# wamuumu/query-recommendation-system

Measured on AMD Instinct MI355X. Metric: MinHash signatures/sec through the whole hot path (signatures -> LSH candidates -> pair scoring -> top-K), higher is better.
Workload: dtype u16/int32 MinHash values, uint64 keys and pairs (integer); float64 cosine

## Files before the change

### include/qrlsh.h

```cpp
#ifndef QRLSH_H
#define QRLSH_H

#include <stddef.h>
#include <stdint.h>

#ifdef __cplusplus
extern "C" {
#endif

#define QRLSH_OK 0
#define QRLSH_EINVAL (-1)
#define QRLSH_EHIP (-2)
#define QRLSH_EUNSUPPORTED (-3)
#define QRLSH_EWORKSPACE (-4)

#define QRLSH_PERM_U16 0
#define QRLSH_PERM_I32 1

#define QRLSH_SIG_I32 0
#define QRLSH_SIG_U16 1

#define QRLSH_SORT_MIX 1u
#define QRLSH_SORT_IOTA 2u
#define QRLSH_SORT_FOLD 4u
// ... 63 lines not shown
int qrlsh_region_unique_count(const uint64_t *grouped, int64_t n, int32_t group_bits, int32_t id_bits, int64_t nids,
                              uint64_t *tmp, void *workspace, size_t workspace_bytes, uint64_t *total_overflow_out,
                              void *stream);
int qrlsh_region_unique_fill(const uint64_t *tmp, int64_t n, int32_t group_bits, int64_t nids, const void *workspace,
                             uint64_t *out, void *stream);

size_t qrlsh_pair_regions_words(int64_t n, int64_t nids, int32_t group_bits, double words_per_query);
size_t qrlsh_pair_regions_tmp_words(int64_t n, int64_t nids, int32_t group_bits, double words_per_query);
int64_t qrlsh_pair_regions_cap(int64_t n, int64_t nids, int32_t group_bits, double words_per_query);
int64_t qrlsh_pair_regions_count(int64_t n, int64_t nids, int32_t group_bits, double words_per_query);
int qrlsh_pair_regions_scatter(const uint64_t *words, int64_t n, int32_t group_bits, int64_t nids, double words_per_query,
                               uint64_t *tmp_regions, uint64_t *regions, uint32_t *counts, uint32_t *overflow_out,
                               void *stream);
int qrlsh_region_unique_count_regions(const uint64_t *regions, const uint32_t *counts, int64_t cap, int64_t n,
                                      int32_t group_bits, int32_t id_bits, int64_t nids, uint64_t *tmp, void *workspace,
                                      size_t workspace_bytes, uint64_t *total_overflow_out, void *stream);
int qrlsh_region_unique_count_regions3(const uint64_t *regions, const uint32_t *counts, int64_t cap, int64_t n,
                                       int32_t group_bits, int32_t id_bits, int64_t nids, uint64_t *tmp, void *workspace,
                                       size_t workspace_bytes, const uint32_t *scatter_overflow, uint64_t *out3,
                                       void *stream);
int qrlsh_pair_regions_scatter32(const uint64_t *words, int64_t n, int32_t group_bits, int32_t id_bits, int64_t nids,
                                 double words_per_query, uint64_t *tmp_regions, uint32_t *regions, uint32_t *counts,
                                 uint32_t *overflow_out, void *stream);
int qrlsh_region_unique_count_regions32(const uint32_t *regions, const uint32_t *counts, int64_t cap, int64_t n,
                                        int32_t group_bits, int32_t id_bits, int64_t nids, uint64_t *tmp, void *workspace,
                                        size_t workspace_bytes, const uint32_t *scatter_overflow, uint64_t *out3,
                                        void *stream);

int qrlsh_row_norms(const int32_t *sig, int64_t nq, int32_t P, int64_t *norm2_out, void *stream);
int qrlsh_verify_pairs(const void *sig, int32_t sig_dtype, int32_t P, int32_t b, const uint64_t *pairs,
                       int64_t n, uint8_t *flags_out, void *stream);
int qrlsh_score_pairs(const void *sig, int32_t sig_dtype, const int64_t *norm2, int32_t P,
                      const uint64_t *pairs, int64_t n, int32_t *milli_out, double *cos_out,
                      uint64_t *edge_out, int32_t id_bits, uint32_t *edge_dst_out, void *stream);

int qrlsh_topk_count(const uint64_t *sorted_edges, int64_t n_edges, int32_t K, int32_t id_bits,
                     void *workspace, size_t workspace_bytes, uint64_t *total_out, void *stream);
int qrlsh_topk_fill(const uint64_t *sorted_edges, const uint32_t *sorted_dst, int64_t n_edges, int32_t K,
                    int32_t id_bits, const void *workspace, int32_t *src_out, int32_t *dst_out,
                    int32_t *milli_out, void *stream);
int qrlsh_topk_fill_based(const uint64_t *sorted_edges, const uint32_t *sorted_dst, int64_t n_edges, int32_t K,
                          int32_t id_bits, int64_t src_base, const void *workspace, int32_t *src_out,
                          int32_t *dst_out, int32_t *milli_out, void *stream);

int qrlsh_score_pairs_rev(const void *sig, int32_t sig_dtype, const int64_t *norm2, int32_t P,
                          const uint64_t *pairs, int64_t n, int32_t *milli_out, uint64_t *rev_out, int32_t id_bits,
// ... 113 lines not shown
```

### query-recommendation-system_amd/csrc/sort.hip

```cpp
#include "common.h"

constexpr int SORT_THREADS = 256;
constexpr int SORT_IPT = 16;
constexpr int SORT_TILE = SORT_THREADS * SORT_IPT;
constexpr int RADIX = 256;

__device__ static inline int xcd_tile(int bid, int ntiles) {
  const int q = ntiles >> 3, r = ntiles & 7, x = bid & 7, y = bid >> 3;
  return (x < r ? x * (q + 1) : r * (q + 1) + (x - r) * q) + y;
}

enum { SM_PLAIN = 0, SM_MIX = 1, SM_FOLD = 2, SM_OWNER = 3, SM_HOST = 4 };
template <int MODE> __device__ static inline uint32_t digit_of(uint64_t key, int shift, uint32_t fold = 0) {
  if (MODE == SM_OWNER || MODE == SM_HOST) {
    const uint64_t o = MODE == SM_HOST ? qr_pair_host(key, fold) : (key >> shift) / fold;
    return o < RADIX ? (uint32_t)o : RADIX - 1;
  }
  uint64_t x = key;
  if (MODE == SM_MIX) x = qr_mix64(key);
  if (MODE == SM_FOLD) x = ((key >> 32) << fold) | (key & ((1ull << fold) - 1ull));
  return (uint32_t)(x >> shift) & (RADIX - 1);
}

template <int MIX>
// ... 304 lines not shown
  const int ntile = (int)min((int64_t)SORT_TILE, n - tbase);
#pragma unroll
  for (int k = 0; k < SORT_IPT; ++k) {
    const int p = k * SORT_THREADS + threadIdx.x;
    if (p < ntile) {
      const uint64_t kk = skey[p];
      keys_out[boff + gdelta[digit_of<MODE>(kk, shift, fold)] + (uint32_t)p] = kk;
    }
  }
}

struct PartPool {
  uint64_t *keys;
  uint32_t *vals;
  unsigned long long *cursor;
  uint32_t cap;
  uint4 *runs;
  unsigned long long *nruns;
  uint32_t runs_max;
  uint32_t *fill;
  uint32_t slot_base;
};

#ifndef QR_PS_IPT
#define QR_PS_IPT 16
#endif
constexpr int PS_IPT = QR_PS_IPT;
constexpr int PS_TILE = SORT_THREADS * PS_IPT;
constexpr int PS_WGS = PS_IPT <= 16 ? 3 : 2;
template <bool LEVEL2>
__global__ __launch_bounds__(SORT_THREADS, PS_WGS) void part_scatter_atomic_kernel(
    const uint64_t *__restrict__ keys_in, const uint32_t *__restrict__ vals_in, uint64_t *__restrict__ keys_out,
    uint32_t *__restrict__ vals_out, int64_t n_in, int ntiles, int shift, uint32_t dmask,
    uint32_t *__restrict__ cursors, uint32_t cap, uint32_t *__restrict__ overflow, uint64_t ek,
    const uint32_t *__restrict__ in_counts, uint32_t in_cap, int64_t chunk_len, int64_t chunk_stride,
    int64_t band_stride, PartPool pool) {
  __shared__ uint32_t cnt[RADIX];
  __shared__ uint32_t lsum[SORT_THREADS / WAVE];
  __shared__ uint32_t gdelta[RADIX];
  __shared__ uint8_t gok[RADIX];
  __shared__ uint64_t skey[PS_TILE];
  __shared__ uint32_t sval[PS_TILE];
  const int tile = LEVEL2 ? (int)blockIdx.x : xcd_tile(blockIdx.x, ntiles), batch = blockIdx.y;
  const int lane = threadIdx.x & (WAVE - 1), w = threadIdx.x >> 6;
  const int64_t n = LEVEL2 ? (int64_t)min(in_counts[batch], in_cap) : n_in;
  const int64_t tbase = (int64_t)tile * PS_TILE;
  if (tbase >= n) return;
  cnt[threadIdx.x] = 0;
  __syncthreads();
  const size_t boff = LEVEL2 ? (size_t)batch * in_cap : (size_t)batch * (size_t)(band_stride ? band_stride : n);
  const bool chunked = !LEVEL2 && chunk_len > 0 && chunk_len < n;
  const int64_t wbase = tbase + (int64_t)w * (WAVE * PS_IPT);
  const uint32_t nd = dmask + 1u;
  uint64_t key[PS_IPT];
  uint32_t val[PS_IPT];
  uint32_t dr[PS_IPT];
#pragma unroll
  for (int k = 0; k < PS_IPT; ++k) {
    const int64_t idx = wbase + (int64_t)k * WAVE + lane;
    const size_t at = chunked ? boff + (size_t)(idx / chunk_len) * chunk_stride + (size_t)(idx % chunk_len) : boff + idx;
    key[k] = idx < n ? keys_in[at] : ek;
    val[k] = LEVEL2 ? (idx < n ? vals_in[boff + idx] : 0u) : (uint32_t)idx;
  }
#pragma unroll
  for (int k = 0; k < PS_IPT; ++k) {
    const int64_t idx = wbase + (int64_t)k * WAVE + lane;
    const bool valid = idx < n && (LEVEL2 || key[k] != ek);
    if (!LEVEL2) key[k] = qr_mix64(key[k]);
    const uint32_t d = (uint32_t)(key[k] >> shift) & dmask;
    dr[k] = valid ? (d << 16) | atomicAdd(&cnt[d], 1u) : 0xFFFFFFFFu;
  }
  __syncthreads();
  const uint32_t tc = cnt[threadIdx.x];
  const uint32_t gb = tc ? atomicAdd(&cursors[(size_t)batch * nd + threadIdx.x], tc) : 0u;
  uint32_t lstart;
  {
    uint32_t linc = tc;
#pragma unroll
    for (int k = 1; k < WAVE; k <<= 1) {
      const uint32_t lo = __shfl_up(linc, k, WAVE);
      if (lane >= k) linc += lo;
    }
    if (lane == WAVE - 1) lsum[w] = linc;
    __syncthreads();
    lstart = linc - tc;
#pragma unroll
    for (int k = 0; k < SORT_THREADS / WAVE; ++k)
      if (k < w) lstart += lsum[k];
    cnt[threadIdx.x] = lstart;
  }
  __syncthreads();
#pragma unroll
  for (int k = 0; k < PS_IPT; ++k) {
    if (dr[k] != 0xFFFFFFFFu) {
      const uint32_t lp = cnt[dr[k] >> 16] + (dr[k] & 0xFFFFu);
      skey[lp] = key[k];
      sval[lp] = val[k];
    }
  }
  {
    const int d = threadIdx.x;
    uint32_t where = gb + tc <= cap ? 1u : 0u;
    uint32_t delta = (uint32_t)d * cap + gb - lstart;
    if (!where) {
      if (pool.keys) {
        const unsigned long long pb =
            __hip_atomic_fetch_add(pool.cursor, (unsigned long long)tc, __ATOMIC_RELAXED, __HIP_MEMORY_SCOPE_AGENT);
        if (pb + tc <= (unsigned long long)pool.cap) {
          const unsigned long long ri = __hip_atomic_fetch_add(pool.nruns, 1ull, __ATOMIC_RELAXED, __HIP_MEMORY_SCOPE_AGENT);
          if (ri < (unsigned long long)pool.runs_max) {
            const uint32_t slot = pool.slot_base + (uint32_t)batch * nd + (uint32_t)d;
            pool.runs[ri] = make_uint4(slot, tc, (uint32_t)pb, 0u);
            atomicMin(&pool.fill[slot], gb);
            where = 2u;
            delta = (uint32_t)pb - lstart;
          }
        }
      }
      if (!where) atomicOr(overflow, 1u);
    }
    gok[d] = (uint8_t)where;
    gdelta[d] = delta;
  }
  __syncthreads();
  uint32_t nstaged = 0;
#pragma unroll
  for (int k = 0; k < SORT_THREADS / WAVE; ++k) nstaged += lsum[k];
  const size_t obase = (size_t)batch * nd * cap;
#pragma unroll
  for (int k = 0; k < PS_IPT; ++k) {
    const uint32_t p = k * SORT_THREADS + threadIdx.x;
    if (p < nstaged) {
      const uint64_t x = skey[p];
      const uint32_t d = (uint32_t)(x >> shift) & dmask;
      const uint32_t where = gok[d];
      if (where == 1u) {
        const size_t dst = obase + (uint32_t)(gdelta[d] + p);
        keys_out[dst] = x;
        vals_out[dst] = sval[p];
      } else if (where == 2u) {
        const uint32_t dst = gdelta[d] + p;
        pool.keys[dst] = x;
        pool.vals[dst] = sval[p];
      }
    }
  }
}

#ifndef QR_PG_IPT
#define QR_PG_IPT 32
#endif
constexpr int PG_IPT = QR_PG_IPT;
constexpr int PG_TILE = SORT_THREADS * PG_IPT;
constexpr int PG_WGS = PG_IPT <= 16 ? 4 : PG_IPT <= 40 ? 2 : 1;
template <bool LEVEL2, typename W>
__global__ __launch_bounds__(SORT_THREADS, PG_WGS) void pair_group_scatter_kernel(
    const uint64_t *__restrict__ in, W *__restrict__ out, int64_t n_in, int ntiles, int shift, uint32_t dmask,
    uint32_t *__restrict__ cursors, uint32_t cap, uint32_t *__restrict__ overflow, const uint32_t *__restrict__ in_counts,
    uint32_t in_cap, int gbits, int jbits) {
  __shared__ uint32_t cnt[RADIX];
  __shared__ uint32_t lsum[SORT_THREADS / WAVE];
  __shared__ uint32_t gdelta[RADIX];
  __shared__ uint8_t gok[RADIX];
  __shared__ uint64_t skey[PG_TILE];
  const int tile = LEVEL2 ? (int)blockIdx.x : xcd_tile(blockIdx.x, ntiles), batch = blockIdx.y;
  const int lane = threadIdx.x & (WAVE - 1), w = threadIdx.x >> 6;
  const int64_t n = LEVEL2 ? (int64_t)min(in_counts[batch], in_cap) : n_in;
  const int64_t tbase = (int64_t)tile * PG_TILE;
  if (tbase >= n) return;
  cnt[threadIdx.x] = 0;
  __syncthreads();
  const size_t boff = LEVEL2 ? (size_t)batch * in_cap : 0;
  const int64_t wbase = tbase + (int64_t)w * (WAVE * PG_IPT);
  const uint32_t nd = dmask + 1u;
  uint64_t key[PG_IPT];
  uint32_t dr[PG_IPT];
#pragma unroll
  for (int k = 0; k < PG_IPT; ++k) {
    const int64_t idx = wbase + (int64_t)k * WAVE + lane;
    key[k] = idx < n ? in[boff + idx] : 0ull;
  }
#pragma unroll
  for (int k = 0; k < PG_IPT; ++k) {
    const int64_t idx = wbase + (int64_t)k * WAVE + lane;
    const uint32_t d = (uint32_t)(key[k] >> shift) & dmask;
    dr[k] = idx < n ? (d << 16) | atomicAdd(&cnt[d], 1u) : 0xFFFFFFFFu;
  }
  __syncthreads();
  const uint32_t tc = cnt[threadIdx.x];
  const uint32_t gb = tc ? atomicAdd(&cursors[(size_t)batch * nd + threadIdx.x], tc) : 0u;
  uint32_t lstart;
  {
    uint32_t linc = tc;
#pragma unroll
    for (int k = 1; k < WAVE; k <<= 1) {
      const uint32_t lo = __shfl_up(linc, k, WAVE);
      if (lane >= k) linc += lo;
    }
    if (lane == WAVE - 1) lsum[w] = linc;
    __syncthreads();
    lstart = linc - tc;
#pragma unroll
    for (int k = 0; k < SORT_THREADS / WAVE; ++k)
      if (k < w) lstart += lsum[k];
    cnt[threadIdx.x] = lstart;
  }
  __syncthreads();
#pragma unroll
  for (int k = 0; k < PG_IPT; ++k)
    if (dr[k] != 0xFFFFFFFFu) skey[cnt[dr[k] >> 16] + (dr[k] & 0xFFFFu)] = key[k];
  {
    const int d = threadIdx.x;
    const bool ok = (uint64_t)gb + tc <= cap;
    if (!ok) atomicOr(overflow, 1u);
    gok[d] = ok;
    gdelta[d] = (uint32_t)d * cap + gb - lstart;
  }
  __syncthreads();
  uint32_t nstaged = 0;
#pragma unroll
  for (int k = 0; k < SORT_THREADS / WAVE; ++k) nstaged += lsum[k];
  const size_t obase = (size_t)batch * nd * cap;
#pragma unroll
  for (int k = 0; k < PG_IPT; ++k) {
    const uint32_t p = k * SORT_THREADS + threadIdx.x;
    if (p < nstaged) {
      const uint64_t x = skey[p];
      const uint32_t d = (uint32_t)(x >> shift) & dmask;
      if (gok[d]) {
        if constexpr (sizeof(W) == 4)
          out[obase + (uint32_t)(gdelta[d] + p)] =
              (((uint32_t)(x >> 32) & ((1u << gbits) - 1u)) << jbits) | ((uint32_t)x & ((1u << jbits) - 1u));
        else
          out[obase + (uint32_t)(gdelta[d] + p)] = x;
      }
    }
  }
}

struct PairRegions {
  int rbits, ra, rb;
  int64_t nregions;
  int64_t na;
  uint32_t cap_a, cap_b;
};
static PairRegions pair_regions(int64_t n, int64_t nids, int group_bits, double words_per_query) {
  PairRegions r;
  const int64_t nr = (nids + (1ll << group_bits) - 1) >> group_bits;
  r.rbits = 1;
  while ((1ll << r.rbits) < nr) ++r.rbits;
  r.rb = r.rbits <= 8 ? r.rbits : (r.rbits + 1) / 2;
  r.ra = r.rbits - r.rb;
  r.na = (nr + (1ll << r.rb) - 1) >> r.rb;
  r.nregions = r.na << r.rb;
  double per = (double)n / (double)(nr > 0 ? nr : 1);
  const double hint = words_per_query * (double)(1ll << group_bits);
  if (hint > per) per = hint;
  const double cb = 3.0 * per + 4096.0;
  const double ca = r.ra ? 2.5 * per * (double)(1ll << r.rb) + 65536.0 : 0.0;
  r.cap_b = (uint32_t)(cb > 4.0e9 ? 4.0e9 : cb);
// ... 30 lines not shown

template <typename W>
static int pair_regions_scatter_impl(const uint64_t *words, int64_t n, int32_t group_bits, int32_t id_bits, int64_t nids,
                                     double words_per_query, uint64_t *tmp_regions, W *regions, uint32_t *counts,
                                     uint32_t *overflow_out, void *stream) {
  QR_CHECK_ARG(n >= 0 && n < (1ll << 32) && nids > 0 && group_bits >= 0 && group_bits <= 8 && counts && overflow_out,
               "qrlsh_pair_regions_scatter: bad arguments");
  hipStream_t st = static_cast<hipStream_t>(stream);
  const PairRegions r = pair_regions(n > 0 ? n : 1, nids, group_bits, words_per_query);
  QR_CHECK_ARG(r.rbits <= 16 && r.na <= RADIX, "qrlsh_pair_regions_scatter: %d region bits", r.rbits);
  QR_CHECK_ARG(pair_regions_fit_u32(r),
               "qrlsh_pair_regions_scatter: regions reach 2^32 words (na * cap_a = %llu, 2^rb * cap_b = %llu; need both < 2^32)",
               (unsigned long long)r.na * r.cap_a, (unsigned long long)r.cap_b << r.rb);
  if (hipMemsetAsync(counts, 0, ((size_t)r.nregions + RADIX) * sizeof(uint32_t), st) != hipSuccess ||
      hipMemsetAsync(overflow_out, 0, sizeof(uint32_t), st) != hipSuccess) {
    qrlsh_set_error("qrlsh_pair_regions_scatter: hipMemsetAsync failed");
    return QRLSH_EHIP;
  }
  if (n == 0) return QRLSH_OK;
  QR_CHECK_ARG(words && regions && (r.ra == 0 || tmp_regions), "qrlsh_pair_regions_scatter: null pointer");
  const int ntiles = (int)ceil_div64(n, PG_TILE);
  const int sh = 32 + group_bits;
  if (r.ra == 0) {
    QR_LAUNCH("pair_group", (pair_group_scatter_kernel<false, W>), dim3(ntiles, 1), dim3(SORT_THREADS), 0, st, words, regions, n,
              ntiles, sh, (1u << r.rb) - 1u, counts, r.cap_b, overflow_out, (const uint32_t *)nullptr, 0u, (int)group_bits,
              (int)id_bits);
  } else {
    uint32_t *cur_a = counts + r.nregions;
    QR_LAUNCH("pair_group", (pair_group_scatter_kernel<false, uint64_t>), dim3(ntiles, 1), dim3(SORT_THREADS), 0, st, words,
              tmp_regions, n, ntiles, sh + r.rb, (1u << r.ra) - 1u, cur_a, r.cap_a, overflow_out, (const uint32_t *)nullptr, 0u,
              0, 0);
    QR_LAUNCH("pair_group", (pair_group_scatter_kernel<true, W>), dim3((unsigned)ceil_div64(r.cap_a, PG_TILE), (unsigned)r.na),
              dim3(SORT_THREADS), 0, st, (const uint64_t *)tmp_regions, regions, (int64_t)0, 0, sh, (1u << r.rb) - 1u, counts,
              r.cap_b, overflow_out, (const uint32_t *)cur_a, r.cap_a, (int)group_bits, (int)id_bits);
  }
  QR_LAUNCH_CHECK("qrlsh_pair_regions_scatter");
  return QRLSH_OK;
}

QRLSH_EXPORT int qrlsh_pair_regions_scatter(const uint64_t *words, int64_t n, int32_t group_bits, int64_t nids,
                                            double words_per_query, uint64_t *tmp_regions, uint64_t *regions,
                                            uint32_t *counts, uint32_t *overflow_out, void *stream) {
  return pair_regions_scatter_impl<uint64_t>(words, n, group_bits, 0, nids, words_per_query, tmp_regions, regions, counts,
                                             overflow_out, stream);
}

QRLSH_EXPORT int qrlsh_pair_regions_scatter32(const uint64_t *words, int64_t n, int32_t group_bits, int32_t id_bits,
                                              int64_t nids, double words_per_query, uint64_t *tmp_regions, uint32_t *regions,
                                              uint32_t *counts, uint32_t *overflow_out, void *stream) {
  QR_CHECK_ARG(group_bits >= 0 && group_bits <= 8 && id_bits >= 1 && id_bits <= 31 && nids > 0 && nids <= (1ll << id_bits) &&
                   (group_bits + id_bits < 32 || (group_bits + id_bits == 32 && nids < (1ll << id_bits))),
               "qrlsh_pair_regions_scatter32: group_bits=%d / id_bits=%d / nids=%lld do not fit a 32-bit value", group_bits,
               id_bits, (long long)nids);
  return pair_regions_scatter_impl<uint32_t>(words, n, group_bits, id_bits, nids, words_per_query, tmp_regions, regions,
                                             counts, overflow_out, stream);
}
// ... 902 lines not shown
  pool.cap = (uint32_t)pool_records(nq, b);
  pool.runs = w.runs;
  pool.runs_max = POOL_RUNS;
  pool.fill = w.fill;
  pool.slot_base = 0;
  PartPool no_pool = pool;
  no_pool.keys = nullptr;
  no_pool.vals = nullptr;
  if (hipMemsetAsync(w.fill, 0xFF, ((size_t)b << T) * sizeof(uint32_t), st) != hipSuccess ||
      hipMemsetAsync(w.poolctl, 0, 16, st) != hipSuccess) {
    qrlsh_set_error("qrlsh_bucket_pairs_emit: hipMemsetAsync failed");
    return QRLSH_EHIP;
  }
  constexpr int MAX_GROUPS = EMIT_MAX_GROUPS;
  unsigned long long *nbig0 = reinterpret_cast<unsigned long long *>(w.big);
  uint64_t *biglist0 = w.big + MAX_GROUPS;
  const uint64_t slots = (uint64_t)b << T;
  if (hipMemsetAsync(nbig0, 0, MAX_GROUPS * sizeof(unsigned long long), st) != hipSuccess) {
    qrlsh_set_error("qrlsh_bucket_pairs_emit: hipMemsetAsync failed");
    return QRLSH_EHIP;
  }
  const bool small_parts = two && small_form(nq, T);
  const int ntiles = (int)ceil_div64(nq, PS_TILE);
  const int64_t band_words = key_band_stride ? key_band_stride : nq;
  const int GROUPS = (int64_t)b * nq >= (64ll << 20) ? MAX_GROUPS : 1;
  const int per = (b + GROUPS - 1) / GROUPS;
  const int ngroups = (b + per - 1) / per;
  const uint64_t list_room = (slots - MAX_GROUPS) / (uint64_t)ngroups;
  const uint32_t big_max = (uint32_t)(list_room < FIN_BIG_LIST ? list_room : FIN_BIG_LIST);
  if (ngroups > 1 && hipMemsetAsync(w.runs, 0, (size_t)POOL_RUNS * sizeof(uint4), st) != hipSuccess) {
    qrlsh_set_error("qrlsh_bucket_pairs_emit: hipMemsetAsync failed");
    return QRLSH_EHIP;
  }
  hipStream_t aux = nullptr;
  int gi = 0;
  for (int g0 = 0; g0 < b; g0 += per, ++gi) {
    const int nb = (b - g0 < per) ? b - g0 : per;
    hipStream_t s = (aux && (gi & 1)) ? aux : st;
    uint64_t *biglist = biglist0 + (size_t)gi * big_max;
    unsigned long long *nbig = nbig0 + gi;
    uint64_t *k1 = two ? tmp_keys : part_keys;
    uint32_t *v1 = two ? tmp_ids : part_ids;
    pool.slot_base = (uint32_t)((size_t)g0 << T);
    BigDesc *desc = w.desc + (size_t)gi * FIN_BIG_LIST;
    QR_PART_SCATTER(false, dim3(ntiles, nb), dim3(SORT_THREADS), 0, s, keys + (size_t)g0 * band_words,
                    (const uint32_t *)nullptr, k1 + ((size_t)g0 << c1) * cap1, v1 + ((size_t)g0 << c1) * cap1, nq,
                    ntiles, 64 - c1, (1u << c1) - 1u, cur1 + ((size_t)g0 << c1), cap1, ovf, qr_empty_key(r),
                    (const uint32_t *)nullptr, 0u, key_chunk, key_chunk_stride, key_band_stride, two ? no_pool : pool);
    if (two)
      QR_PART_SCATTER(true, dim3((unsigned)ceil_div64(cap1, PS_TILE), nb << c1), dim3(SORT_THREADS), 0, s,
                      (const uint64_t *)tmp_keys + ((size_t)g0 << c1) * cap1,
                      (const uint32_t *)tmp_ids + ((size_t)g0 << c1) * cap1, part_keys + ((size_t)g0 << T) * cap2,
                      part_ids + ((size_t)g0 << T) * cap2, (int64_t)0, 0, 64 - T, lowmask, cur2 + ((size_t)g0 << T),
                      cap2, ovf, qr_empty_key(r), (const uint32_t *)cur1 + ((size_t)g0 << c1), cap1, (int64_t)0,
                      (int64_t)0, (int64_t)0, pool);
    if (gi == 0 && b > per) aux = qr_aux_fork(st);
    if (small_parts && T >= 12)
      QR_LAUNCH("bucket_emit", bucket_finish_packed_kernel, dim3(nparts, nb), dim3(FIN_PK_THREADS), 0, s,
                (const uint64_t *)part_keys + ((size_t)g0 << T) * cap2, (const uint32_t *)part_ids + ((size_t)g0 << T) * cap2,
                nparts, total_overflow_out, ovf, pairs_out, capacity, (const uint32_t *)cur2 + ((size_t)g0 << T), cap2, biglist,
                nbig, big_max, (uint32_t)((size_t)g0 << T));
    else if (small_parts)
      QR_LAUNCH("bucket_emit", (bucket_finish_kernel<FIN_SMALL_THREADS, FIN_SMALL_CAP>), dim3(nparts, nb),
                dim3(FIN_SMALL_THREADS), 0, s, (const uint64_t *)part_keys + ((size_t)g0 << T) * cap2,
                (const uint32_t *)part_ids + ((size_t)g0 << T) * cap2, nparts, ekx,
                total_overflow_out, ovf, pairs_out, capacity, (const uint32_t *)cur2 + ((size_t)g0 << T), cap2, biglist, nbig,
                big_max, (uint32_t)((size_t)g0 << T));
    else
      QR_LAUNCH("bucket_emit", (bucket_finish_kernel<>), dim3(nparts, nb), dim3(FIN_THREADS), 0, s,
                (const uint64_t *)part_keys + ((size_t)g0 << T) * cap2, (const uint32_t *)part_ids + ((size_t)g0 << T) * cap2,
                nparts, ekx, total_overflow_out, ovf, pairs_out, capacity,
                (const uint32_t *)cur2 + ((size_t)g0 << T), cap2, biglist, nbig, big_max, (uint32_t)((size_t)g0 << T));
    QR_LAUNCH("bucket_emit_big", bucket_big_gather_kernel, dim3(64), dim3(256), 0, s, (const uint64_t *)biglist,
              (const unsigned long long *)nbig, big_max, desc, (const uint64_t *)part_keys, (const uint32_t *)part_ids,
              (const uint32_t *)cur2, cap2, pool, g_big_limit, ovf);
    QR_LAUNCH("bucket_emit_big", bucket_finish_big_kernel, dim3(FIN_BIG_GRID), dim3(FIN_THREADS), 0, s,
// ... 10 lines not shown
```

### query-recommendation-system_amd/qrlsh/_lib.py

```python
import ctypes
import os

_HERE = os.path.dirname(os.path.abspath(__file__))
LIB_PATH = os.environ.get("QRLSH_LIB", os.path.join(_HERE, "libqrlsh.so"))

QRLSH_OK = 0
QRLSH_EINVAL = -1
QRLSH_EHIP = -2
QRLSH_EUNSUPPORTED = -3
QRLSH_EWORKSPACE = -4

PERM_U16 = 0
PERM_I32 = 1
SIG_I32 = 0
SIG_U16 = 1
SORT_MIX = 1
SORT_IOTA = 2
SORT_FOLD = 4
SORT_OWNER = 8
SORT_HOST = 16
SUM_PAIRWISE = 0
SUM_SEQUENTIAL = 1
RECOMMEND_MAX_K = 1024
INDEX_MAX_K = 256
# ... 23 lines not shown
    "qrlsh_bucket_part_words": (_sz, [_i64, _i32, _i32]),
    "qrlsh_set_big_part_limit": (_i64, [_i64]),
    "qrlsh_set_score_runs": (_i32, [_i32]),
    "qrlsh_bucket_tmp_words": (_sz, [_i64, _i32, _i32]),
    "qrlsh_bucket_pairs_emit": (ctypes.c_int, [_vp, _vp, _vp, _vp, _vp, _i64, _i32, _i32, _i32, _vp, _sz, _vp, _u64, _vp, _vp]),
    "qrlsh_compact_workspace_bytes": (_sz, [_i64]),
    "qrlsh_row_unique_workspace_bytes": (_sz, [_i64]),
    "qrlsh_row_unique_count": (ctypes.c_int, [_vp, _i64, _i32, _i32, _vp, _vp, _sz, _vp, _vp]),
    "qrlsh_row_unique_fill": (ctypes.c_int, [_vp, _i64, _vp, _vp, _vp]),
    "qrlsh_region_unique_workspace_bytes": (_sz, [_i64, _i32]),
    "qrlsh_region_unique_count": (ctypes.c_int, [_vp, _i64, _i32, _i32, _i64, _vp, _vp, _sz, _vp, _vp]),
    "qrlsh_region_unique_fill": (ctypes.c_int, [_vp, _i64, _i32, _i64, _vp, _vp, _vp]),
    "qrlsh_region_unique_count_regions": (ctypes.c_int, [_vp, _vp, _i64, _i64, _i32, _i32, _i64, _vp, _vp, _sz, _vp, _vp]),
    "qrlsh_region_unique_count_regions3": (ctypes.c_int, [_vp, _vp, _i64, _i64, _i32, _i32, _i64, _vp, _vp, _sz, _vp, _vp,
                                                          _vp]),
    "qrlsh_region_unique_count_regions32": (ctypes.c_int, [_vp, _vp, _i64, _i64, _i32, _i32, _i64, _vp, _vp, _sz, _vp, _vp,
                                                           _vp]),
    "qrlsh_pair_regions_scatter32": (ctypes.c_int, [_vp, _i64, _i32, _i32, _i64, ctypes.c_double, _vp, _vp, _vp, _vp, _vp]),
    "qrlsh_pair_regions_words": (_sz, [_i64, _i64, _i32, ctypes.c_double]),
    "qrlsh_pair_regions_tmp_words": (_sz, [_i64, _i64, _i32, ctypes.c_double]),
    "qrlsh_pair_regions_cap": (_i64, [_i64, _i64, _i32, ctypes.c_double]),
    "qrlsh_pair_regions_count": (_i64, [_i64, _i64, _i32, ctypes.c_double]),
    "qrlsh_pair_regions_scatter": (ctypes.c_int, [_vp, _i64, _i32, _i64, ctypes.c_double, _vp, _vp, _vp, _vp, _vp]),
    "qrlsh_unique_count": (ctypes.c_int, [_vp, _i64, _vp, _sz, _vp, _vp]),
    "qrlsh_unique_fill": (ctypes.c_int, [_vp, _i64, _vp, _vp, _vp]),
    "qrlsh_row_norms": (ctypes.c_int, [_vp, _i64, _i32, _vp, _vp]),
    "qrlsh_verify_pairs": (ctypes.c_int, [_vp, _i32, _i32, _i32, _vp, _i64, _vp, _vp]),
    "qrlsh_score_pairs": (ctypes.c_int, [_vp, _i32, _vp, _i32, _vp, _i64, _vp, _vp, _vp, _i32, _vp, _vp]),
    "qrlsh_remap_pairs": (ctypes.c_int, [_vp, _i64, _i64, _i64, _vp, _i64, _vp, _vp]),
    "qrlsh_pair_edges": (ctypes.c_int, [_vp, _vp, _i64, _i32, _vp, _vp, _vp, _vp, _vp]),
    "qrlsh_topk_count": (ctypes.c_int, [_vp, _i64, _i32, _i32, _vp, _sz, _vp, _vp]),
    "qrlsh_topk_fill": (ctypes.c_int, [_vp, _vp, _i64, _i32, _i32, _vp, _vp, _vp, _vp, _vp]),
    "qrlsh_topk_fill_based": (ctypes.c_int, [_vp, _vp, _i64, _i32, _i32, _i64, _vp, _vp, _vp, _vp, _vp]),
    "qrlsh_score_pairs_rev": (ctypes.c_int, [_vp, _i32, _vp, _i32, _vp, _i64, _vp, _vp, _i32, _vp, _vp]),
    "qrlsh_topk_select_workspace_bytes": (_sz, [_i64]),
    "qrlsh_topk_select_count": (ctypes.c_int, [_vp, _i64, _vp, _vp, _i64, _i32, _i32, _vp, _sz, _vp, _vp]),
    "qrlsh_topk_select_fill": (ctypes.c_int, [_vp, _vp, _i64, _vp, _vp, _i64, _i32, _i32, _vp, _vp, _vp, _vp, _vp]),
    "qrlsh_idset_workspace_bytes": (_sz, [_i64]),
    "qrlsh_idset_build": (ctypes.c_int, [_vp, _i64, _i64, _i64, _i64, _i64, _i32, _vp, _sz, _vp, _vp]),
    "qrlsh_idset_list": (ctypes.c_int, [_vp, _i64, _vp, _vp]),
    "qrlsh_idset_remap": (ctypes.c_int, [_vp, _i64, _i64, _i64, _vp, _i64, _vp, _vp]),
    "qrlsh_gather_rows": (ctypes.c_int, [_vp, _i64, _vp, _vp, _i64, _i64, _vp, _vp, _vp]),
    "qrlsh_score_pairs_split": (ctypes.c_int, [_vp, _vp, _i64, _vp, _vp, _i32, _i32, _vp, _i64, _vp, _vp]),
    "qrlsh_edges_localize": (ctypes.c_int, [_vp, _vp, _i64, _i32, _i64, _i64, _vp, _vp]),
    "qrlsh_answer_sets_count": (ctypes.c_int, [_vp, _i64, _i64, _vp, _i64, _i32, _vp, _vp]),
    "qrlsh_answer_sets_fill": (ctypes.c_int, [_vp, _i64, _i64, _vp, _i64, _i32, _vp, _vp, _vp]),
# ... 87 lines not shown
```

Before: 619.4 million.

## Make partition scatter kernels persistent with a prefetched next tile

Changes the partition-scatter and pair-group-scatter kernels from one block per (tile, batch) to a persistent grid sized from occupancy queries. Each block walks tiles with an XCD-aware stride, skips empty level-2 tiles, and loads the next tile's keys into registers while it scatters the current tile. This is meant to cut launch and block-retire overhead, avoid launching blocks for empty level-2 tiles, and hide global load latency. In exchange it adds loop control, extra barriers and higher register pressure, and it exposes a tile-grid query to Python.

New measurement: 612.4 million. 1.1% lower.

```diff
diff --git a/include/qrlsh.h b/include/qrlsh.h
--- a/include/qrlsh.h
+++ b/include/qrlsh.h
@@ -109,6 +109,7 @@
 int qrlsh_pair_regions_scatter32(const uint64_t *words, int64_t n, int32_t group_bits, int32_t id_bits, int64_t nids,
                                  double words_per_query, uint64_t *tmp_regions, uint32_t *regions, uint32_t *counts,
                                  uint32_t *overflow_out, void *stream);
+int32_t qrlsh_tile_grid(int32_t family, int32_t *tile_records_out);
 int qrlsh_region_unique_count_regions32(const uint32_t *regions, const uint32_t *counts, int64_t cap, int64_t n,
                                         int32_t group_bits, int32_t id_bits, int64_t nids, uint64_t *tmp, void *workspace,
                                         size_t workspace_bytes, const uint32_t *scatter_overflow, uint64_t *out3,
diff --git a/query-recommendation-system_amd/csrc/sort.hip b/query-recommendation-system_amd/csrc/sort.hip
--- a/query-recommendation-system_amd/csrc/sort.hip
+++ b/query-recommendation-system_amd/csrc/sort.hip
@@ -1,4 +1,5 @@
 #include "common.h"
+#include <atomic>
 
 constexpr int SORT_THREADS = 256;
 constexpr int SORT_IPT = 16;
@@ -350,6 +351,43 @@
   uint32_t slot_base;
 };
 
+struct TileWalk {
+  uint32_t pos, stride, len, start, end;
+};
+template <bool LEVEL2> __device__ static inline TileWalk walk_init(int ntiles, int nbatch) {
+  TileWalk wk;
+  if (LEVEL2) {
+    wk.pos = blockIdx.x;
+    wk.stride = gridDim.x;
+    wk.len = (uint32_t)ntiles;
+    wk.start = 0;
+  } else {
+    const uint32_t q = (uint32_t)ntiles >> 3, r = (uint32_t)ntiles & 7u, x = blockIdx.x & 7u;
+    wk.len = q + (x < r ? 1u : 0u);
+    wk.start = x < r ? x * (q + 1u) : r * (q + 1u) + (x - r) * q;
+    wk.pos = blockIdx.x >> 3;
+    wk.stride = (gridDim.x - x + 7u) >> 3;
+  }
+  wk.end = (uint32_t)nbatch * wk.len;
+  return wk;
+}
+template <bool LEVEL2>
+__device__ static inline bool walk_seek(TileWalk &wk, int tile_len, int64_t n_in, const uint32_t *__restrict__ in_counts,
+                                        uint32_t in_cap, int &batch, int &tile, int64_t &n) {
+  while (wk.pos < wk.end) {
+    const uint32_t bt = wk.pos / wk.len, t = wk.pos - bt * wk.len;
+    n = LEVEL2 ? (int64_t)min(in_counts[bt], in_cap) : n_in;
+    if (!LEVEL2 || (int64_t)t * tile_len < n) {
+      batch = (int)bt;
+      tile = (int)(wk.start + t);
+      return true;
+    }
+    const uint32_t gap = (bt + 1u) * wk.len - wk.pos;
+    wk.pos += (gap + wk.stride - 1u) / wk.stride * wk.stride;
+  }
+  return false;
+}
+
 #ifndef QR_PS_IPT
 #define QR_PS_IPT 16
 #endif
@@ -359,7 +397,7 @@
 template <bool LEVEL2>
 __global__ __launch_bounds__(SORT_THREADS, PS_WGS) void part_scatter_atomic_kernel(
     const uint64_t *__restrict__ keys_in, const uint32_t *__restrict__ vals_in, uint64_t *__restrict__ keys_out,
-    uint32_t *__restrict__ vals_out, int64_t n_in, int ntiles, int shift, uint32_t dmask,
+    uint32_t *__restrict__ vals_out, int64_t n_in, int ntiles, int nbatch, int shift, uint32_t dmask,
     uint32_t *__restrict__ cursors, uint32_t cap, uint32_t *__restrict__ overflow, uint64_t ek,
     const uint32_t *__restrict__ in_counts, uint32_t in_cap, int64_t chunk_len, int64_t chunk_stride,
     int64_t band_stride, PartPool pool) {
@@ -369,67 +407,78 @@
   __shared__ uint8_t gok[RADIX];
   __shared__ uint64_t skey[PS_TILE];
   __shared__ uint32_t sval[PS_TILE];
-  const int tile = LEVEL2 ? (int)blockIdx.x : xcd_tile(blockIdx.x, ntiles), batch = blockIdx.y;
   const int lane = threadIdx.x & (WAVE - 1), w = threadIdx.x >> 6;
-  const int64_t n = LEVEL2 ? (int64_t)min(in_counts[batch], in_cap) : n_in;
-  const int64_t tbase = (int64_t)tile * PS_TILE;
-  if (tbase >= n) return;
-  cnt[threadIdx.x] = 0;
-  __syncthreads();
-  const size_t boff = LEVEL2 ? (size_t)batch * in_cap : (size_t)batch * (size_t)(band_stride ? band_stride : n);
-  const bool chunked = !LEVEL2 && chunk_len > 0 && chunk_len < n;
-  const int64_t wbase = tbase + (int64_t)w * (WAVE * PS_IPT);
   const uint32_t nd = dmask + 1u;
+  const bool chunked = !LEVEL2 && chunk_len > 0 && chunk_len < n_in;
+  TileWalk wk = walk_init<LEVEL2>(ntiles, nbatch);
+  int batch, tile;
+  int64_t n;
+  if (!walk_seek<LEVEL2>(wk, PS_TILE, n_in, in_counts, in_cap, batch, tile, n)) return;
   uint64_t key[PS_IPT];
   uint32_t val[PS_IPT];
   uint32_t dr[PS_IPT];
-#pragma unroll
-  for (int k = 0; k < PS_IPT; ++k) {
-    const int64_t idx = wbase + (int64_t)k * WAVE + lane;
-    const size_t at = chunked ? boff + (size_t)(idx / chunk_len) * chunk_stride + (size_t)(idx % chunk_len) : boff + idx;
-    key[k] = idx < n ? keys_in[at] : ek;
-    val[k] = LEVEL2 ? (idx < n ? vals_in[boff + idx] : 0u) : (uint32_t)idx;
-  }
-#pragma unroll
-  for (int k = 0; k < PS_IPT; ++k) {
-    const int64_t idx = wbase + (int64_t)k * WAVE + lane;
-    const bool valid = idx < n && (LEVEL2 || key[k] != ek);
-    if (!LEVEL2) key[k] = qr_mix64(key[k]);
-    const uint32_t d = (uint32_t)(key[k] >> shift) & dmask;
-    dr[k] = valid ? (d << 16) | atomicAdd(&cnt[d], 1u) : 0xFFFFFFFFu;
-  }
-  __syncthreads();
-  const uint32_t tc = cnt[threadIdx.x];
-  const uint32_t gb = tc ? atomicAdd(&cursors[(size_t)batch * nd + threadIdx.x], tc) : 0u;
-  uint32_t lstart;
-  {
-    uint32_t linc = tc;
-#pragma unroll
-    for (int k = 1; k < WAVE; k <<= 1) {
-      const uint32_t lo = __shfl_up(linc, k, WAVE);
-      if (lane >= k) linc += lo;
-    }
-    if (lane == WAVE - 1) lsum[w] = linc;
-    __syncthreads();
-    lstart = linc - tc;
-#pragma unroll
-    for (int k = 0; k < SORT_THREADS / WAVE; ++k)
-      if (k < w) lstart += lsum[k];
-    cnt[threadIdx.x] = lstart;
-  }
-  __syncthreads();
-#pragma unroll
-  for (int k = 0; k < PS_IPT; ++k) {
-    if (dr[k] != 0xFFFFFFFFu) {
-      const uint32_t lp = cnt[dr[k] >> 16] + (dr[k] & 0xFFFFu);
-      skey[lp] = key[k];
-      sval[lp] = val[k];
-    }
-  }
-  {
+  auto load_tile = [&](int bt, int tl, int64_t nn) {
+    const size_t boff = LEVEL2 ? (size_t)bt * in_cap : (size_t)bt * (size_t)(band_stride ? band_stride : nn);
+    const int64_t wbase = (int64_t)tl * PS_TILE + (int64_t)w * (WAVE * PS_IPT);
+#pragma unroll
+    for (int k = 0; k < PS_IPT; ++k) {
+      const int64_t idx = wbase + (int64_t)k * WAVE + lane;
+      const size_t at = chunked ? boff + (size_t)(idx / chunk_len) * chunk_stride + (size_t)(idx % chunk_len) : boff + idx;
+      key[k] = idx < nn ? keys_in[at] : ek;
+      val[k] = LEVEL2 ? (idx < nn ? vals_in[boff + idx] : 0u) : (uint32_t)idx;
+    }
+  };
+  load_tile(batch, tile, n);
+  cnt[threadIdx.x] = 0;
+  __syncthreads();
+  for (;;) {
+    const int64_t wbase = (int64_t)tile * PS_TILE + (int64_t)w * (WAVE * PS_IPT);
+#pragma unroll
+    for (int k = 0; k < PS_IPT; ++k) {
+      const int64_t idx = wbase + (int64_t)k * WAVE + lane;
+      const bool valid = idx < n && (LEVEL2 || key[k] != ek);
+      if (!LEVEL2) key[k] = qr_mix64(key[k]);
+      const uint32_t d = (uint32_t)(key[k] >> shift) & dmask;
+      dr[k] = valid ? (d << 16) | atomicAdd(&cnt[d], 1u) : 0xFFFFFFFFu;
+    }
+    __syncthreads();
+    const uint32_t tc = cnt[threadIdx.x];
+    const uint32_t gb = tc ? atomicAdd(&cursors[(size_t)batch * nd + threadIdx.x], tc) : 0u;
+    uint32_t lstart;
+    {
+      uint32_t linc = tc;
+#pragma unroll
+      for (int k = 1; k < WAVE; k <<= 1) {
+        const uint32_t lo = __shfl_up(linc, k, WAVE);
+        if (lane >= k) linc += lo;
+      }
+      if (lane == WAVE - 1) lsum[w] = linc;
+      __syncthreads();
+      lstart = linc - tc;
+#pragma unroll
+      for (int k = 0; k < SORT_THREADS / WAVE; ++k)
+        if (k < w) lstart += lsum[k];
+      cnt[threadIdx.x] = lstart;
+    }
+    __syncthreads();
+#pragma unroll
+    for (int k = 0; k < PS_IPT; ++k) {
+      if (dr[k] != 0xFFFFFFFFu) {
+        const uint32_t lp = cnt[dr[k] >> 16] + (dr[k] & 0xFFFFu);
+        skey[lp] = key[k];
+        sval[lp] = val[k];
+      }
+    }
     const int d = threadIdx.x;
     uint32_t where = gb + tc <= cap ? 1u : 0u;
     uint32_t delta = (uint32_t)d * cap + gb - lstart;
+    gok[d] = (uint8_t)where;
+    gdelta[d] = delta;
+    int nbt, ntl;
+    int64_t nn;
+    wk.pos += wk.stride;
+    const bool more = walk_seek<LEVEL2>(wk, PS_TILE, n_in, in_counts, in_cap, nbt, ntl, nn);
+    if (more) load_tile(nbt, ntl, nn);
     if (!where) {
       if (pool.keys) {
         const unsigned long long pb =
@@ -446,32 +495,38 @@
         }
       }
       if (!where) atomicOr(overflow, 1u);
-    }
-    gok[d] = (uint8_t)where;
-    gdelta[d] = delta;
-  }
-  __syncthreads();
-  uint32_t nstaged = 0;
-#pragma unroll
-  for (int k = 0; k < SORT_THREADS / WAVE; ++k) nstaged += lsum[k];
-  const size_t obase = (size_t)batch * nd * cap;
-#pragma unroll
-  for (int k = 0; k < PS_IPT; ++k) {
-    const uint32_t p = k * SORT_THREADS + threadIdx.x;
-    if (p < nstaged) {
-      const uint64_t x = skey[p];
-      const uint32_t d = (uint32_t)(x >> shift) & dmask;
-      const uint32_t where = gok[d];
-      if (where == 1u) {
-        const size_t dst = obase + (uint32_t)(gdelta[d] + p);
-        keys_out[dst] = x;
-        vals_out[dst] = sval[p];
-      } else if (where == 2u) {
-        const uint32_t dst = gdelta[d] + p;
-        pool.keys[dst] = x;
-        pool.vals[dst] = sval[p];
-      }
-    }
+      gok[d] = (uint8_t)where;
+      gdelta[d] = delta;
+    }
+    __syncthreads();
+    cnt[threadIdx.x] = 0;
+    uint32_t nstaged = 0;
+#pragma unroll
+    for (int k = 0; k < SORT_THREADS / WAVE; ++k) nstaged += lsum[k];
+    const size_t obase = (size_t)batch * nd * cap;
+#pragma unroll
+    for (int k = 0; k < PS_IPT; ++k) {
+      const uint32_t p = k * SORT_THREADS + threadIdx.x;
+      if (p < nstaged) {
+        const uint64_t x = skey[p];
+        const uint32_t d = (uint32_t)(x >> shift) & dmask;
+        const uint32_t where = gok[d];
+        if (where == 1u) {
+          const size_t dst = obase + (uint32_t)(gdelta[d] + p);
+          keys_out[dst] = x;
+          vals_out[dst] = sval[p];
+        } else if (where == 2u) {
+          const uint32_t dst = gdelta[d] + p;
+          pool.keys[dst] = x;
+          pool.vals[dst] = sval[p];
+        }
+      }
+    }
+    if (!more) break;
+    __syncthreads();
+    batch = nbt;
+    tile = ntl;
+    n = nn;
   }
 }
 
@@ -483,7 +538,7 @@
 constexpr int PG_WGS = PG_IPT <= 16 ? 4 : PG_IPT <= 40 ? 2 : 1;
 template <bool LEVEL2, typename W>
 __global__ __launch_bounds__(SORT_THREADS, PG_WGS) void pair_group_scatter_kernel(
-    const uint64_t *__restrict__ in, W *__restrict__ out, int64_t n_in, int ntiles, int shift, uint32_t dmask,
+    const uint64_t *__restrict__ in, W *__restrict__ out, int64_t n_in, int ntiles, int nbatch, int shift, uint32_t dmask,
     uint32_t *__restrict__ cursors, uint32_t cap, uint32_t *__restrict__ overflow, const uint32_t *__restrict__ in_counts,
     uint32_t in_cap, int gbits, int jbits) {
   __shared__ uint32_t cnt[RADIX];
@@ -491,79 +546,133 @@
   __shared__ uint32_t gdelta[RADIX];
   __shared__ uint8_t gok[RADIX];
   __shared__ uint64_t skey[PG_TILE];
-  const int tile = LEVEL2 ? (int)blockIdx.x : xcd_tile(blockIdx.x, ntiles), batch = blockIdx.y;
   const int lane = threadIdx.x & (WAVE - 1), w = threadIdx.x >> 6;
-  const int64_t n = LEVEL2 ? (int64_t)min(in_counts[batch], in_cap) : n_in;
-  const int64_t tbase = (int64_t)tile * PG_TILE;
-  if (tbase >= n) return;
-  cnt[threadIdx.x] = 0;
-  __syncthreads();
-  const size_t boff = LEVEL2 ? (size_t)batch * in_cap : 0;
-  const int64_t wbase = tbase + (int64_t)w * (WAVE * PG_IPT);
   const uint32_t nd = dmask + 1u;
+  TileWalk wk = walk_init<LEVEL2>(ntiles, nbatch);
+  int batch, tile;
+  int64_t n;
+  if (!walk_seek<LEVEL2>(wk, PG_TILE, n_in, in_counts, in_cap, batch, tile, n)) return;
   uint64_t key[PG_IPT];
   uint32_t dr[PG_IPT];
-#pragma unroll
-  for (int k = 0; k < PG_IPT; ++k) {
-    const int64_t idx = wbase + (int64_t)k * WAVE + lane;
-    key[k] = idx < n ? in[boff + idx] : 0ull;
-  }
-#pragma unroll
-  for (int k = 0; k < PG_IPT; ++k) {
-    const int64_t idx = wbase + (int64_t)k * WAVE + lane;
-    const uint32_t d = (uint32_t)(key[k] >> shift) & dmask;
-    dr[k] = idx < n ? (d << 16) | atomicAdd(&cnt[d], 1u) : 0xFFFFFFFFu;
-  }
-  __syncthreads();
-  const uint32_t tc = cnt[threadIdx.x];
-  const uint32_t gb = tc ? atomicAdd(&cursors[(size_t)batch * nd + threadIdx.x], tc) : 0u;
-  uint32_t lstart;
-  {
-    uint32_t linc = tc;
-#pragma unroll
-    for (int k = 1; k < WAVE; k <<= 1) {
-      const uint32_t lo = __shfl_up(linc, k, WAVE);
-      if (lane >= k) linc += lo;
-    }
-    if (lane == WAVE - 1) lsum[w] = linc;
-    __syncthreads();
-    lstart = linc - tc;
-#pragma unroll
-    for (int k = 0; k < SORT_THREADS / WAVE; ++k)
-      if (k < w) lstart += lsum[k];
-    cnt[threadIdx.x] = lstart;
-  }
-  __syncthreads();
-#pragma unroll
-  for (int k = 0; k < PG_IPT; ++k)
-    if (dr[k] != 0xFFFFFFFFu) skey[cnt[dr[k] >> 16] + (dr[k] & 0xFFFFu)] = key[k];
-  {
-    const int d = threadIdx.x;
-    const bool ok = (uint64_t)gb + tc <= cap;
-    if (!ok) atomicOr(overflow, 1u);
-    gok[d] = ok;
-    gdelta[d] = (uint32_t)d * cap + gb - lstart;
-  }
-  __syncthreads();
-  uint32_t nstaged = 0;
-#pragma unroll
-  for (int k = 0; k < SORT_THREADS / WAVE; ++k) nstaged += lsum[k];
-  const size_t obase = (size_t)batch * nd * cap;
-#pragma unroll
-  for (int k = 0; k < PG_IPT; ++k) {
-    const uint32_t p = k * SORT_THREADS + threadIdx.x;
-    if (p < nstaged) {
-      const uint64_t x = skey[p];
-      const uint32_t d = (uint32_t)(x >> shift) & dmask;
-      if (gok[d]) {
-        if constexpr (sizeof(W) == 4)
-          out[obase + (uint32_t)(gdelta[d] + p)] =
-              (((uint32_t)(x >> 32) & ((1u << gbits) - 1u)) << jbits) | ((uint32_t)x & ((1u << jbits) - 1u));
-        else
-          out[obase + (uint32_t)(gdelta[d] + p)] = x;
-      }
-    }
-  }
+  auto load_tile = [&](int bt, int tl, int64_t nn) {
+    const size_t boff = LEVEL2 ? (size_t)bt * in_cap : 0;
+    const int64_t wbase = (int64_t)tl * PG_TILE + (int64_t)w * (WAVE * PG_IPT);
+#pragma unroll
+    for (int k = 0; k < PG_IPT; ++k) {
+      const int64_t idx = wbase + (int64_t)k * WAVE + lane;
+      key[k] = idx < nn ? in[boff + idx] : 0ull;
+    }
+  };
+  load_tile(batch, tile, n);
+  cnt[threadIdx.x] = 0;
+  __syncthreads();
+  for (;;) {
+    const int64_t wbase = (int64_t)tile * PG_TILE + (int64_t)w * (WAVE * PG_IPT);
+#pragma unroll
+    for (int k = 0; k < PG_IPT; ++k) {
+      const int64_t idx = wbase + (int64_t)k * WAVE + lane;
+      const uint32_t d = (uint32_t)(key[k] >> shift) & dmask;
+      dr[k] = idx < n ? (d << 16) | atomicAdd(&cnt[d], 1u) : 0xFFFFFFFFu;
+    }
+    __syncthreads();
+    const uint32_t tc = cnt[threadIdx.x];
+    const uint32_t gb = tc ? atomicAdd(&cursors[(size_t)batch * nd + threadIdx.x], tc) : 0u;
+    uint32_t lstart;
+    {
+      uint32_t linc = tc;
+#pragma unroll
+      for (int k = 1; k < WAVE; k <<= 1) {
+        const uint32_t lo = __shfl_up(linc, k, WAVE);
+        if (lane >= k) linc += lo;
+      }
+      if (lane == WAVE - 1) lsum[w] = linc;
+      __syncthreads();
+      lstart = linc - tc;
+#pragma unroll
+      for (int k = 0; k < SORT_THREADS / WAVE; ++k)
+        if (k < w) lstart += lsum[k];
+      cnt[threadIdx.x] = lstart;
+    }
+    __syncthreads();
+#pragma unroll
+    for (int k = 0; k < PG_IPT; ++k)
+      if (dr[k] != 0xFFFFFFFFu) skey[cnt[dr[k] >> 16] + (dr[k] & 0xFFFFu)] = key[k];
+    {
+      const int d = threadIdx.x;
+      const bool ok = (uint64_t)gb + tc <= cap;
+      if (!ok) atomicOr(overflow, 1u);
+      gok[d] = ok;
+      gdelta[d] = (uint32_t)d * cap + gb - lstart;
+    }
+    int nbt, ntl;
+    int64_t nn;
+    wk.pos += wk.stride;
+    const bool more = walk_seek<LEVEL2>(wk, PG_TILE, n_in, in_counts, in_cap, nbt, ntl, nn);
+    if (more) load_tile(nbt, ntl, nn);
+    __syncthreads();
+    cnt[threadIdx.x] = 0;
+    uint32_t nstaged = 0;
+#pragma unroll
+    for (int k = 0; k < SORT_THREADS / WAVE; ++k) nstaged += lsum[k];
+    const size_t obase = (size_t)batch * nd * cap;
+#pragma unroll
+    for (int k = 0; k < PG_IPT; ++k) {
+      const uint32_t p = k * SORT_THREADS + threadIdx.x;
+      if (p < nstaged) {
+        const uint64_t x = skey[p];
+        const uint32_t d = (uint32_t)(x >> shift) & dmask;
+        if (gok[d]) {
+          if constexpr (sizeof(W) == 4)
+            out[obase + (uint32_t)(gdelta[d] + p)] =
+                (((uint32_t)(x >> 32) & ((1u << gbits) - 1u)) << jbits) | ((uint32_t)x & ((1u << jbits) - 1u));
+          else
+            out[obase + (uint32_t)(gdelta[d] + p)] = x;
+        }
+      }
+    }
+    if (!more) break;
+    __syncthreads();
+    batch = nbt;
+    tile = ntl;
+    n = nn;
+  }
+}
+
+static int tile_grid_resident(int family) {
+  static std::atomic<int> cache[2][16];
+  int dev = 0;
+  if (hipGetDevice(&dev) != hipSuccess || dev < 0 || dev >= 16) dev = 0;
+  int g = cache[family][dev].load(std::memory_order_relaxed);
+  if (g > 0) return g;
+  hipDeviceProp_t prop;
+  int cus = 256;
+  if (hipGetDeviceProperties(&prop, dev) == hipSuccess && prop.multiProcessorCount > 0) cus = prop.multiProcessorCount;
+  const void *kerns[2][4] = {
+      {(const void *)part_scatter_atomic_kernel<false>, (const void *)part_scatter_atomic_kernel<true>, nullptr, nullptr},
+      {(const void *)pair_group_scatter_kernel<false, uint64_t>, (const void *)pair_group_scatter_kernel<true, uint64_t>,
+       (const void *)pair_group_scatter_kernel<false, uint32_t>, (const void *)pair_group_scatter_kernel<true, uint32_t>}};
+  int per_cu = family == 0 ? PS_WGS : PG_WGS;
+  int least = 0;
+  for (int i = 0; i < 4; ++i) {
+    int nb = 0;
+    if (kerns[family][i] && hipOccupancyMaxActiveBlocksPerMultiprocessor(&nb, kerns[family][i], SORT_THREADS, 0) == hipSuccess &&
+        nb > 0 && (least == 0 || nb < least))
+      least = nb;
+  }
+  (void)hipGetLastError();
+  if (least > 0) per_cu = least;
+  g = cus * per_cu;
+  cache[family][dev].store(g, std::memory_order_relaxed);
+  return g;
+}
+static unsigned tile_grid(int family, int64_t items) {
+  const int64_t g = tile_grid_resident(family);
+  return (unsigned)(items < g ? (items > 0 ? items : 1) : g);
+}
+QRLSH_EXPORT int32_t qrlsh_tile_grid(int32_t family, int32_t *tile_records_out) {
+  if (family != 0 && family != 1) return 0;
+  if (tile_records_out) *tile_records_out = family == 0 ? PS_TILE : PG_TILE;
+  return tile_grid_resident(family);
 }
 
 struct PairRegions {
@@ -640,16 +749,17 @@
   const int ntiles = (int)ceil_div64(n, PG_TILE);
   const int sh = 32 + group_bits;
   if (r.ra == 0) {
-    QR_LAUNCH("pair_group", (pair_group_scatter_kernel<false, W>), dim3(ntiles, 1), dim3(SORT_THREADS), 0, st, words, regions, n,
-              ntiles, sh, (1u << r.rb) - 1u, counts, r.cap_b, overflow_out, (const uint32_t *)nullptr, 0u, (int)group_bits,
+    QR_LAUNCH("pair_group", (pair_group_scatter_kernel<false, W>), dim3(tile_grid(1, ntiles)), dim3(SORT_THREADS), 0, st, words, regions, n,
+              ntiles, 1, sh, (1u << r.rb) - 1u, counts, r.cap_b, overflow_out, (const uint32_t *)nullptr, 0u, (int)group_bits,
               (int)id_bits);
   } else {
     uint32_t *cur_a = counts + r.nregions;
-    QR_LAUNCH("pair_group", (pair_group_scatter_kernel<false, uint64_t>), dim3(ntiles, 1), dim3(SORT_THREADS), 0, st, words,
-              tmp_regions, n, ntiles, sh + r.rb, (1u << r.ra) - 1u, cur_a, r.cap_a, overflow_out, (const uint32_t *)nullptr, 0u,
+    QR_LAUNCH("pair_group", (pair_group_scatter_kernel<false, uint64_t>), dim3(tile_grid(1, ntiles)), dim3(SORT_THREADS), 0, st, words,
+              tmp_regions, n, ntiles, 1, sh + r.rb, (1u << r.ra) - 1u, cur_a, r.cap_a, overflow_out, (const uint32_t *)nullptr, 0u,
               0, 0);
-    QR_LAUNCH("pair_group", (pair_group_scatter_kernel<true, W>), dim3((unsigned)ceil_div64(r.cap_a, PG_TILE), (unsigned)r.na),
-              dim3(SORT_THREADS), 0, st, (const uint64_t *)tmp_regions, regions, (int64_t)0, 0, sh, (1u << r.rb) - 1u, counts,
+    const int tiles_a = (int)ceil_div64(r.cap_a, PG_TILE);
+    QR_LAUNCH("pair_group", (pair_group_scatter_kernel<true, W>), dim3(tile_grid(1, (int64_t)tiles_a * r.na)),
+              dim3(SORT_THREADS), 0, st, (const uint64_t *)tmp_regions, regions, (int64_t)0, tiles_a, (int)r.na, sh, (1u << r.rb) - 1u, counts,
               r.cap_b, overflow_out, (const uint32_t *)cur_a, r.cap_a, (int)group_bits, (int)id_bits);
   }
   QR_LAUNCH_CHECK("qrlsh_pair_regions_scatter");
@@ -1598,6 +1708,9 @@
   }
   const bool small_parts = two && small_form(nq, T);
   const int ntiles = (int)ceil_div64(nq, PS_TILE);
+  const int tiles1 = (int)ceil_div64(cap1, PS_TILE);
+  QR_CHECK_ARG((int64_t)ntiles * b < (1ll << 31) && ((int64_t)tiles1 * b << c1) < (1ll << 31),
+               "qrlsh_bucket_pairs_emit: %lld x %d tiles", (long long)ntiles, b);
   const int64_t band_words = key_band_stride ? key_band_stride : nq;
   const int GROUPS = (int64_t)b * nq >= (64ll << 20) ? MAX_GROUPS : 1;
   const int per = (b + GROUPS - 1) / GROUPS;
@@ -1619,15 +1732,15 @@
     uint32_t *v1 = two ? tmp_ids : part_ids;
     pool.slot_base = (uint32_t)((size_t)g0 << T);
     BigDesc *desc = w.desc + (size_t)gi * FIN_BIG_LIST;
-    QR_PART_SCATTER(false, dim3(ntiles, nb), dim3(SORT_THREADS), 0, s, keys + (size_t)g0 * band_words,
+    QR_PART_SCATTER(false, dim3(tile_grid(0, (int64_t)ntiles * nb)), dim3(SORT_THREADS), 0, s, keys + (size_t)g0 * band_words,
                     (const uint32_t *)nullptr, k1 + ((size_t)g0 << c1) * cap1, v1 + ((size_t)g0 << c1) * cap1, nq,
-                    ntiles, 64 - c1, (1u << c1) - 1u, cur1 + ((size_t)g0 << c1), cap1, ovf, qr_empty_key(r),
+                    ntiles, nb, 64 - c1, (1u << c1) - 1u, cur1 + ((size_t)g0 << c1), cap1, ovf, qr_empty_key(r),
                     (const uint32_t *)nullptr, 0u, key_chunk, key_chunk_stride, key_band_stride, two ? no_pool : pool);
     if (two)
-      QR_PART_SCATTER(true, dim3((unsigned)ceil_div64(cap1, PS_TILE), nb << c1), dim3(SORT_THREADS), 0, s,
+      QR_PART_SCATTER(true, dim3(tile_grid(0, (int64_t)tiles1 * (nb << c1))), dim3(SORT_THREADS), 0, s,
                       (const uint64_t *)tmp_keys + ((size_t)g0 << c1) * cap1,
                       (const uint32_t *)tmp_ids + ((size_t)g0 << c1) * cap1, part_keys + ((size_t)g0 << T) * cap2,
-                      part_ids + ((size_t)g0 << T) * cap2, (int64_t)0, 0, 64 - T, lowmask, cur2 + ((size_t)g0 << T),
+                      part_ids + ((size_t)g0 << T) * cap2, (int64_t)0, tiles1, nb << c1, 64 - T, lowmask, cur2 + ((size_t)g0 << T),
                       cap2, ovf, qr_empty_key(r), (const uint32_t *)cur1 + ((size_t)g0 << c1), cap1, (int64_t)0,
                       (int64_t)0, (int64_t)0, pool);
     if (gi == 0 && b > per) aux = qr_aux_fork(st);
diff --git a/query-recommendation-system_amd/qrlsh/_lib.py b/query-recommendation-system_amd/qrlsh/_lib.py
--- a/query-recommendation-system_amd/qrlsh/_lib.py
+++ b/query-recommendation-system_amd/qrlsh/_lib.py
@@ -69,6 +69,7 @@
     "qrlsh_pair_regions_cap": (_i64, [_i64, _i64, _i32, ctypes.c_double]),
     "qrlsh_pair_regions_count": (_i64, [_i64, _i64, _i32, ctypes.c_double]),
     "qrlsh_pair_regions_scatter": (ctypes.c_int, [_vp, _i64, _i32, _i64, ctypes.c_double, _vp, _vp, _vp, _vp, _vp]),
+    "qrlsh_tile_grid": (_i32, [_i32, _vp]),
     "qrlsh_unique_count": (ctypes.c_int, [_vp, _i64, _vp, _sz, _vp, _vp]),
     "qrlsh_unique_fill": (ctypes.c_int, [_vp, _i64, _vp, _vp, _vp]),
     "qrlsh_row_norms": (ctypes.c_int, [_vp, _i64, _i32, _vp, _vp]),
```
